# Circuitscape/Circuitscape.jl

Measured on NVIDIA H100. Metric: pair_solves_per_sec, higher is better.
Workload: dtype f64

## Files before the change

### circuitscape_b200/csrc/cs_b200.cu

```cuda
#include "../../include/cs_b200.h"

#include <cuda_runtime.h>
#include <cub/device/device_scan.cuh>

#include <algorithm>
#include <chrono>
#include <cmath>
#include <cstdarg>
#include <cstdio>
#include <cstdlib>
#include <cstring>
#include <limits>
#include <string>
#include <type_traits>
#include <vector>

#include "amg_host.hpp"
#include "win_host.hpp"
#include "kernels.cuh"
#include "raster_assembly.cuh"
#include "setup_device.hpp"

using namespace csb;

// ... 73 lines not shown
  bool mixed = false;
  std::vector<DevLevel> lv32;
  void *R32 = nullptr, *X32 = nullptr, *T32 = nullptr, *Z32 = nullptr;
  void *d_cum = nullptr, *d_max = nullptr;
  int* d_bptr = nullptr;
  int64_t nb = 0;
  void* d_cum_branch = nullptr;
  void* d_branch_stage = nullptr;
  PanelCtl* d_ctl = nullptr;
  PanelCtl* h_ctl = nullptr;
  double* d_partials = nullptr;
  float* d_flush = nullptr;
  size_t flush_elems = 0;
  cudaStream_t stream = nullptr;
  cudaEvent_t ev0 = nullptr, ev1 = nullptr, ev2 = nullptr, ev3 = nullptr;
  long long* d_sp_rows = nullptr;
  double* d_sp_vals = nullptr;
  int* d_sp_ptr = nullptr;
  size_t sp_cap = 0;
  long long* d_probe = nullptr;
  void* d_probe_out = nullptr;
  size_t probe_cap = 0;
  cudaStream_t s_in = nullptr, s_out = nullptr;
  void* io_in[2] = {nullptr, nullptr};
  void* io_out[2] = {nullptr, nullptr};
  cudaEvent_t ev_in[2] = {nullptr, nullptr}, ev_used[2] = {nullptr, nullptr};
  cudaEvent_t ev_ready[2] = {nullptr, nullptr}, ev_out[2] = {nullptr, nullptr};
  int num_sms = 132;
  int grid_spmm = 132, grid_ew = 132;
  cs_b200_opts opts{};
  cs_b200_stats stats{};
  GraphSlot graphs[4];
  bool rg_on = false;
  int* d_rg_seg = nullptr;
  int* d_rg_rows = nullptr;
  size_t rg_cap = 0;
  GraphSlot rgraphs[4];
  int profile = 0;
  std::vector<cudaEvent_t> prof_ev;
  size_t prof_used = 0;
  double prof_ms = 0.0;
  double prof_bytes = 0.0;
  int64_t prof_launches = 0;
  std::vector<int> prof_slot;
  std::vector<double> prof_pair_bytes;
  double prof_slot_ms[PROF_CLASSES] = {}, prof_slot_bytes[PROF_CLASSES] = {};
  int64_t prof_slot_launches[PROF_CLASSES] = {};
  std::string err;
  size_t esize() const { return dtype == CS_B200_F64 ? 8 : 4; }
};

namespace {

struct Tick {
  bool on = std::getenv("CS_B200_VERBOSE") != nullptr;
  std::chrono::steady_clock::time_point t0 = std::chrono::steady_clock::now();
  void operator()(const char* what) {
    if (!on) return;
    const auto t1 = std::chrono::steady_clock::now();
    std::fprintf(stderr, "[cs_b200 setup] %-28s %8.1f ms\n", what,
                 std::chrono::duration<double, std::milli>(t1 - t0).count());
    t0 = t1;
  }
};

int set_err(cs_b200_handle* h, int code, const char* fmt, ...) {
// ... 676 lines not shown

inline int copy_grid(size_t nelem) { return (int)std::min<size_t>(4096, (nelem + 255) / 256); }

template <typename T, int KT, int MODE, bool HALF>
void launch_stencil_pipe(cs_b200_handle* h, const DiaDev<T>& a, const T* X, T* Y, const SpmmEpi<T>& ep, int sg) {
  constexpr int SMEM = StPipe<T, KT, MODE, HALF>::D::BYTES;
  set_max_smem_once<k_stencil_pipe<T, KT, MODE, HALF>>(h, SMEM);
  k_stencil_pipe<T, KT, MODE, HALF><<<sg, NT, SMEM, h->stream>>>(a, X, Y, ep);
}

template <typename T, int KT, int MODE>
void launch_stencil(cs_b200_handle* h, const DiaDev<T>& a, const T* X, T* Y, const SpmmEpi<T>& ep, int sg) {
  if (!stencil_pipe()) {
    if (a.half) refuse_half("k_stencil");
    k_stencil<T, KT, MODE><<<sg, NT, 0, h->stream>>>(a, X, Y, ep);
    return;
  }
  if (a.half) launch_stencil_pipe<T, KT, MODE, true>(h, a, X, Y, ep, sg);
  else launch_stencil_pipe<T, KT, MODE, false>(h, a, X, Y, ep, sg);
}

template <typename T, int KT, int MODE, bool WIDE>
void launch_spmm_win(cs_b200_handle* h, const DevCsr& m, const T* X, T* Y, const SpmmEpi<T>& ep) {
  constexpr int SMEM = WinSmem2<T, KT, MODE, WIDE>::TOTAL;
  constexpr int SB = WinMap<T, KT, WIDE>::SB;
  const WinCsr<T> w{m.win_meta, m.blob, m.has_dinv, m.rowptr, m.colidx, (const T*)m.vals, m.win_nblocks};
  const int wg = std::max(1, std::min(h->num_sms, (m.win_nblocks + SB - 1) / SB));
  set_max_smem_once<k_spmm_win<T, KT, MODE, WIDE>>(h, SMEM);
  k_spmm_win<T, KT, MODE, WIDE><<<wg, WTT, SMEM, h->stream>>>(w, X, Y, ep);
}

template <typename T, int KT, int MODE>
void launch_spmm_on(cs_b200_handle* h, const DevCsr& m, const T* X, T* Y, const T* B, const T* dinv,
                    double omega, bool timed) {
  const int grid = std::max(1, std::min(h->grid_spmm, m.nblocks));
  double bytes = (double)m.nnz * (sizeof(T) + 4) + (double)(m.nrows + 1) * 4 +
                 2.0 * (double)m.nrows * KT * sizeof(T);
  if (MODE == SP_RESNORM || MODE == SP_RES || MODE == SP_JACOBI || MODE == SP_JACOBI_DOT)
    bytes += (double)m.nrows * KT * sizeof(T);
  if (MODE == SP_JACOBI || MODE == SP_JACOBI_DOT) bytes += (double)m.nrows * sizeof(T);
  const ProfScope prof(h, timed, MODE, sizeof(T) == 4, bytes);
  const SpmmEpi<T> ep{B, dinv, (T)omega, h->d_ctl, h->d_partials};
  if (m.dia && MODE != SP_ADD) {
    if constexpr (MODE != SP_ADD) launch_stencil<T, KT, MODE>(h, dia_view<T>(m), X, Y, ep, stencil_grid<T, KT>(h, m));
  } else if (m.win_meta) {
    if (m.lpr == 4) launch_spmm_win<T, KT, MODE, true>(h, m, X, Y, ep);
    else launch_spmm_win<T, KT, MODE, false>(h, m, X, Y, ep);
  } else if (m.lpr == 4 && KT * 4 <= 32) {
    k_spmm<T, KT, MODE, (KT * 4 <= 32 ? 4 : 1)><<<grid, NT, 0, h->stream>>>(view<T>(m), X, Y, ep);
  } else {
    k_spmm<T, KT, MODE, 1><<<grid, NT, 0, h->stream>>>(view<T>(m), X, Y, ep);
  }
}

template <typename T, int KT, int MODE>
void launch_spmm(cs_b200_handle* h, const T* X, T* Y, const T* B) {
  launch_spmm_on<T, KT, MODE>(h, h->A0, X, Y, B, (const T*)h->d_dinv, 0.0, true);
}

void harvest_profile(cs_b200_handle* h) {
  for (size_t i = 0; i + 1 < h->prof_used; i += 2) {
    float ms = 0;
    if (cudaEventElapsedTime(&ms, h->prof_ev[i], h->prof_ev[i + 1]) == cudaSuccess) {
      h->prof_ms += ms;
      h->prof_launches++;
      if (i / 2 < h->prof_slot.size()) {
        const int sl = h->prof_slot[i / 2];
        h->prof_slot_ms[sl] += ms;
        h->prof_slot_bytes[sl] += h->prof_pair_bytes[i / 2];
        h->prof_slot_launches[sl]++;
      }
    }
  }
  h->prof_used = 0;
  h->prof_slot.clear();
// ... 108 lines not shown

template <typename T, int KT>
void launch_seg_set(cs_b200_handle* h, void* panel, int set_b_only, T v) {
  k_seg_set<T, KT><<<2 * KT, NT, 0, h->stream>>>((T*)panel, h->d_rg_seg, h->d_rg_rows, set_b_only, v);
  h->stats.kernel_launches++;
}

template <typename T, int KT>
void mask_z(cs_b200_handle* h) {
  if (!h->rg_on) return;
  if (h->mixed) launch_seg_set<float, KT>(h, h->Z32, 0, 0.0f);
  else launch_seg_set<T, KT>(h, h->Z, 0, T(0));
}

inline GraphSlot& graph_slot(cs_b200_handle* h, int kt) {
  return (h->rg_on ? h->rgraphs : h->graphs)[kt_index(kt)];
}

void drop_graphs(GraphSlot* slots) {
  for (int i = 0; i < 4; ++i) {
    if (slots[i].exec) cudaGraphExecDestroy(slots[i].exec);
    if (slots[i].loop_exec) cudaGraphExecDestroy(slots[i].loop_exec);
    slots[i] = GraphSlot{};
  }
}

inline bool fused_cg(const cs_b200_handle* h) {
  static const bool off = std::getenv("CS_B200_NO_FUSED_CG") != nullptr;
  return h->amg && h->A0.dia && h->P2 && !off;
}

inline bool fused_res(const cs_b200_handle* h) {
  return fused_cg(h) && h->R2 && !h->rg_on && fused_res_form(h);
}

template <typename T, int KT, typename TV, bool HALF, bool STORE_AP>
void launch_stencil_cg_pipe(cs_b200_handle* h, const DiaDev<T>& a, const TV* Z, int sg) {
  constexpr int SMEM = StPipeCg<T, KT, TV, HALF>::D::BYTES;
  set_max_smem_once<k_stencil_cg_pipe<T, KT, TV, HALF, STORE_AP>>(h, SMEM);
  k_stencil_cg_pipe<T, KT, TV, HALF, STORE_AP><<<sg, NT, SMEM, h->stream>>>(a, Z, (T*)h->P2, (T*)h->P, (T*)h->X,
                                                                            (T*)h->AP, h->d_ctl, h->d_partials);
}

template <typename T, int KT, typename TV>
void launch_stencil_cg(cs_b200_handle* h, const TV* Z, bool store_ap) {
  const DevCsr& m = h->A0;
  const DiaDev<T> a = dia_view<T>(m);
  const int sg = stencil_grid<T, KT>(h, m);
  const double pe = (double)m.nrows * KT * sizeof(T);
  const double fb = (double)m.nrows * 9 * sizeof(T) + (double)m.nrows * KT * sizeof(TV) + (store_ap ? 3.0 : 2.0) * pe +
                    1.5 * pe;
  const ProfScope prof(h, true, PROF_CGF, sizeof(T) == 4, fb);
  if (stencil_pipe()) {
    if (!store_ap) {
      if constexpr (sizeof(T) == 8 && sizeof(TV) == 4) launch_stencil_cg_pipe<T, KT, TV, true, false>(h, a, Z, sg);
    } else if (a.half) launch_stencil_cg_pipe<T, KT, TV, true, true>(h, a, Z, sg);
    else launch_stencil_cg_pipe<T, KT, TV, false, true>(h, a, Z, sg);
  } else {
    if (a.half) refuse_half("k_stencil_cg");
    k_stencil_cg<T, KT, TV><<<sg, NT, 0, h->stream>>>(a, Z, (T*)h->P2, (T*)h->P, (T*)h->X, (T*)h->AP, h->d_ctl,
                                                       h->d_partials);
  }
}

template <typename T, int KT>
void launch_res_update(cs_b200_handle* h) {
// ... 133 lines not shown
    const int64_t kl = h->stats.kernel_launches, sl = h->stats.spmm_launches;
    CK(h, cudaStreamBeginCaptureToGraph(h->stream, body, nullptr, nullptr, 0, cudaStreamCaptureModeThreadLocal));
    launch_iteration<T, KT>(h);
    k_loop_cond<<<1, 1, 0, h->stream>>>(cond, h->d_ctl);
    CK(h, cudaStreamEndCapture(h->stream, nullptr));
    gs.loop_kernels = h->stats.kernel_launches - kl + 1;
    gs.loop_spmms = h->stats.spmm_launches - sl;
    h->stats.kernel_launches = kl;
    h->stats.spmm_launches = sl;
    CK(h, cudaGraphInstantiate(&gs.loop_exec, graph, 0));
    cudaGraphDestroy(graph);
  }
  CK(h, cudaGraphLaunch(gs.loop_exec, h->stream));
  return CS_B200_OK;
}

template <typename T, int KT>
int solve_panel(cs_b200_handle* h, double rtol, int64_t itmax) {
  const size_t nelem = (size_t)h->n_pad * KT;
  const double atol = h->opts.atol > 0 ? h->opts.atol
                      : h->opts.atol < 0 ? 0.0
                      : std::sqrt(std::numeric_limits<double>::epsilon());
  const int g = ew_grid<T, KT>(h);
  const int imax = (int)std::min<int64_t>(itmax, std::numeric_limits<int>::max() - 1);
  CK(h, cudaEventRecord(h->ev2, h->stream));
  if (!h->amg) {
    k_set_stall<<<1, 1, 0, h->stream>>>(h->d_ctl, 2000);
    k_cg_init<T, KT><<<g, NT, 0, h->stream>>>(nelem, (const T*)h->B, (const T*)h->d_dinv, (T*)h->X,
                                              (T*)h->R, (T*)h->P, h->d_ctl, h->d_partials, rtol, atol,
                                              imax);
    h->stats.kernel_launches++;
  } else {
    const bool fused = fused_cg(h);
    CK(h, cudaMemsetAsync(h->X, 0, nelem * sizeof(T), h->stream));
    CK(h, cudaMemsetAsync(h->P, 0, nelem * sizeof(T), h->stream));
    CK(h, cudaMemcpyAsync(h->R, h->B, nelem * sizeof(T), cudaMemcpyDeviceToDevice, h->stream));
    k_set_ctl<<<1, 1, 0, h->stream>>>(h->d_ctl, rtol, atol, imax, 40);
    h->stats.kernel_launches++;
    if (h->mixed) {
      k_convert<T, float><<<g, NT, 0, h->stream>>>(nelem, (const T*)h->R, (float*)h->R32);
      h->stats.kernel_launches++;
    }
    launch_vcycle<T, KT>(h, false);
    mask_z<T, KT>(h);
    if (!fused) launch_update_xp2<T, KT>(h);
  }
  CK(h, cudaGetLastError());
  const int chunk = h->amg ? std::min(h->opts.check_every, 4) : h->opts.check_every;
  const bool device_loop = h->opts.use_graph == 1 && !h->profile;
  if (device_loop) {
    int rc = run_loop<T, KT>(h);
    if (rc) return rc;
  }
  for (;;) {
    CK(h, cudaMemcpyAsync(h->h_ctl, h->d_ctl, sizeof(PanelCtl), cudaMemcpyDeviceToHost, h->stream));
    CK(h, cudaStreamSynchronize(h->stream));
    if (h->profile) harvest_profile(h);
    if (device_loop) {
      GraphSlot& gs = graph_slot(h, KT);
      h->stats.kernel_launches += 1 + gs.loop_kernels * h->h_ctl->iter;
      h->stats.spmm_launches += gs.loop_spmms * h->h_ctl->iter;
      break;
    }
    if (h->h_ctl->nactive == 0) break;
    int rc = run_chunk<T, KT>(h, chunk);
    if (rc) return rc;
  }
  if (h->amg) finish_x<T, KT>(h);
  if (h->rg_on) {
    launch_spmm<T, KT, SP_RES>(h, (const T*)h->X, (T*)h->AP, (const T*)h->B);
    launch_seg_set<T, KT>(h, h->AP, 0, T(0));
    k_resnorm<T, KT><<<g, NT, 0, h->stream>>>(nelem, (size_t)h->n * KT, (const T*)h->AP, (const T*)h->B, h->d_ctl, h->d_partials);
    h->stats.kernel_launches++;
  } else {
    launch_spmm<T, KT, 2>(h, (const T*)h->X, (T*)h->AP, (const T*)h->B);
  }
  CK(h, cudaGetLastError());
  CK(h, cudaEventRecord(h->ev3, h->stream));
  CK(h, cudaMemcpyAsync(h->h_ctl, h->d_ctl, sizeof(PanelCtl), cudaMemcpyDeviceToHost, h->stream));
  CK(h, cudaStreamSynchronize(h->stream));
  if (h->profile) harvest_profile(h);
  float ms = 0;
  CK(h, cudaEventElapsedTime(&ms, h->ev2, h->ev3));
  h->stats.kernel_ms += ms;
  return CS_B200_OK;
}

int next_kt(int64_t remaining, int ktmax) {
  int kt = ktmax;
  while (kt > remaining) kt >>= 1;
  return kt < 1 ? 1 : kt;
}

#define DISPATCH_KT(kt, CALL)                    \
  switch (kt) {                                  \
    case 1: { constexpr int KT = 1; CALL; } break; \
    case 2: { constexpr int KT = 2; CALL; } break; \
    case 4: { constexpr int KT = 4; CALL; } break; \
    default: { constexpr int KT = 8; CALL; } break; \
  }

template <typename F>
decltype(auto) with_type(const cs_b200_handle* h, F&& f) {
  return h->dtype == CS_B200_F64 ? f(double{}) : f(float{});
}

template <typename F>
decltype(auto) with_width(int kt, F&& f) {
  DISPATCH_KT(kt, return f(std::integral_constant<int, KT>{}));
}

template <typename F>
decltype(auto) with_type_width(const cs_b200_handle* h, int kt, F&& f) {
  return with_type(h, [&](auto t) -> decltype(auto) {
    return with_width(kt, [&](auto KT) -> decltype(auto) { return f(t, KT); });
  });
}

struct ColumnDriver {
  cs_b200_handle* h;
  bool any_fail = false, any_maxit = false;
  std::string msg;

  template <typename Panel>
  int run(int64_t c_begin, int64_t c_end, Panel&& panel) {
    for (int64_t c0 = c_begin; c0 < c_end;) {
      const int kt = next_kt(c_end - c0, h->ktmax);
      if (int rc = with_width(kt, [&](auto KT) { return panel(KT, c0); })) return rc;
      c0 += kt;
    }
    return CS_B200_OK;
  }

  template <typename T, int KT>
  int solve(int64_t c0, double rtol, int64_t itmax, int64_t* iters, double* relres, bool masked = false) {
    h->rg_on = masked;
    const int rc = solve_panel<T, KT>(h, rtol, itmax);
    h->rg_on = false;
    if (!rc) gather(KT, c0, iters, relres, itmax);
    return rc;
  }

  void gather(int kt, int64_t c0, int64_t* iters, double* relres, int64_t itmax) {
    for (int c = 0; c < kt; ++c) {
      const PanelCtl& ct = *h->h_ctl;
      const double bn = ct.bnorm[c];
      const double rr = bn > 0 ? std::sqrt(ct.resid[c] / bn) : 0.0;
      if (iters) iters[c0 + c] = ct.iters[c];
      if (relres) relres[c0 + c] = rr;
      h->stats.iterations += ct.iters[c];
      if (!(rr < h->opts.resid_gate)) {
        if (!any_fail) {
          char buf[256];
          snprintf(buf, sizeof buf,
                   "CUDA PCG solver residual %g exceeds tolerance %g for column %lld (%d iterations)",
                   rr, h->opts.resid_gate, (long long)(c0 + c + 1), ct.iters[c]);
          msg = buf;
        }
        any_fail = true;
      }
      if ((ct.iters[c] >= itmax || ct.stalled[c]) && std::sqrt(ct.rho[c]) > ct.tol[c]) any_maxit = true;
    }
  }

  int verdict(int rc) const {
    if (rc) return rc;
    if (any_fail) return set_err(h, CS_B200_ERR_RESIDUAL, "%s", msg.c_str());
    if (any_maxit) return set_err(h, CS_B200_ERR_MAXITER, "itmax reached (or the recurrence stagnated) before rtol");
    return CS_B200_OK;
  }
};
// ... 122 lines not shown
  }
  CK(h, h2d(h, h->d_probe, probe, need * sizeof(long long)));
  return CS_B200_OK;
}

template <typename T, int KT>
int download_outputs(cs_b200_handle* h, int64_t c0, T* curr, T* volt, int volt_shift) {
  CK(h, cudaGetLastError());
  const int tg = copy_grid((size_t)h->n_pad * KT);
  auto download = [&](const void* panel, int shift, T* out) -> int {
    k_panel_to_cm<T, KT><<<tg, 256, 0, h->stream>>>((int)h->n, (size_t)h->n, (const T*)panel, (T*)h->stage,
                                                    h->d_ctl, shift);
    h->stats.kernel_launches++;
    CK(h, cudaMemcpyAsync(out + (size_t)c0 * h->n, h->stage, (size_t)h->n * KT * sizeof(T),
                          cudaMemcpyDeviceToHost, h->stream));
    h->stats.d2h_bytes += (double)h->n * KT * sizeof(T);
    return CS_B200_OK;
  };
  if (curr)
    if (int rc = download(h->AP, 0, curr)) return rc;
  if (volt)
    if (int rc = download(h->X, volt_shift, volt)) return rc;
  return CS_B200_OK;
}

template <typename T, int KT>
int currents_and_outputs(cs_b200_handle* h, int64_t c0, T* curr, T* volt, int accumulate, int volt_shift,
                         const void* fg = nullptr) {
  if (accumulate || curr) launch_currents<T, KT>(h, curr != nullptr, accumulate, fg);
  return download_outputs<T, KT>(h, c0, curr, volt, volt_shift);
}

template <typename T, int KT>
int pairs_panel(cs_b200_handle* h, int64_t c0, const int64_t* src, const int64_t* dst,
                const double* weight, double rtol, int64_t itmax, T* R, T* volt, T* curr,
                int accumulate, int64_t* iters, double* relres, ColumnDriver& cols) {
  if (int rc = upload_ctl(h, KT, [&](int c) {
        return ColCtl{src[c0 + c], dst[c0 + c], col_weight(weight, c0 + c)};
      }))
    return rc;
  CK(h, cudaMemsetAsync(h->B, 0, (size_t)h->n_pad * KT * sizeof(T), h->stream));
  k_pair_rhs<T, KT><<<1, 32, 0, h->stream>>>((T*)h->B, h->d_ctl);
  h->stats.kernel_launches++;
  if (int rc = cols.solve<T, KT>(c0, rtol, itmax, iters, relres)) return rc;
  k_pair_extract<T, KT><<<1, 32, 0, h->stream>>>((const T*)h->X, h->d_ctl);
  h->stats.kernel_launches++;
  if (int rc = currents_and_outputs<T, KT>(h, c0, curr, volt, accumulate, 1)) return rc;
  if (int rc = read_ctl(h)) return rc;
  for (int c = 0; c < KT; ++c) R[c0 + c] = (T)(h->h_ctl->xdst[c] - h->h_ctl->xsrc[c]);
  return CS_B200_OK;
}

template <typename T, int KT>
int sources_panel(cs_b200_handle* h, int64_t c0, const int64_t* colptr, const int64_t* rows,
                  const double* vals, const int64_t* ref, const double* weight, double rtol,
                  int64_t itmax, int64_t nprobe, T* probe_volt, T* volt, T* curr, int accumulate,
                  int64_t* iters, double* relres, ColumnDriver& cols) {
  if (int rc = upload_ctl(h, KT, [&](int c) { return ColCtl{ref[c0 + c], -1, col_weight(weight, c0 + c)}; }))
    return rc;
  if (int rc = upload_sparse_rhs(h, KT, colptr + c0, rows, vals)) return rc;
  CK(h, cudaMemsetAsync(h->B, 0, (size_t)h->n_pad * KT * sizeof(T), h->stream));
  k_sparse_rhs<T, KT><<<1, 32, 0, h->stream>>>((T*)h->B, h->d_sp_ptr, h->d_sp_rows, h->d_sp_vals);
  h->stats.kernel_launches++;
  if (int rc = cols.solve<T, KT>(c0, rtol, itmax, iters, relres)) return rc;
  k_pair_extract<T, KT><<<1, 32, 0, h->stream>>>((const T*)h->X, h->d_ctl);
  h->stats.kernel_launches++;
  if (nprobe > 0 && probe_volt) {
    k_probe<T, KT><<<(int)std::min<int64_t>(64, (nprobe * KT + 255) / 256), 256, 0, h->stream>>>(
        (const T*)h->X, h->d_ctl, h->d_probe, (int)nprobe, (T*)h->d_probe_out);
    h->stats.kernel_launches++;
    CK(h, cudaMemcpyAsync(probe_volt + (size_t)c0 * nprobe, h->d_probe_out, (size_t)nprobe * KT * sizeof(T),
                          cudaMemcpyDeviceToHost, h->stream));
    h->stats.d2h_bytes += (double)nprobe * KT * sizeof(T);
  }
  if (int rc = currents_and_outputs<T, KT>(h, c0, curr, volt, accumulate, 1)) return rc;
  CK(h, cudaStreamSynchronize(h->stream));
  return CS_B200_OK;
}

template <typename T, int KT>
int point_panel(cs_b200_handle* h, int64_t x0, const int64_t* nodes, double rtol, int64_t itmax, T* U,
                int64_t* point_iters, ColumnDriver& cols) {
  const size_t nelem = (size_t)h->n_pad * KT;
  if (int rc = upload_ctl(h, KT, [&](int c) { return ColCtl{nodes[0], nodes[x0 + c], 1.0}; })) return rc;
  CK(h, cudaMemsetAsync(h->B, 0, nelem * sizeof(T), h->stream));
  k_pair_rhs<T, KT><<<1, 32, 0, h->stream>>>((T*)h->B, h->d_ctl);
  h->stats.kernel_launches++;
  if (int rc = cols.solve<T, KT>(0, rtol, itmax, nullptr, nullptr)) return rc;
  if (point_iters)
    for (int c = 0; c < KT; ++c) point_iters[x0 - 1 + c] = h->h_ctl->iters[c];
  k_pair_extract<T, KT><<<1, 32, 0, h->stream>>>((const T*)h->X, h->d_ctl);
  const int tg = copy_grid(nelem);
  k_panel_to_cm<T, KT><<<tg, 256, 0, h->stream>>>((int)h->n, (size_t)h->n_pad, (const T*)h->X,
                                                  U + (size_t)(x0 - 1) * h->n_pad, h->d_ctl, 1);
  h->stats.kernel_launches += 2;
  CK(h, cudaGetLastError());
  CK(h, cudaStreamSynchronize(h->stream));
  return CS_B200_OK;
}

template <typename T, int KT>
int combine_panel(cs_b200_handle* h, int64_t c0, const int64_t* nodes, const int64_t* pi, const int64_t* pj,
                  const double* weight, const T* U, int* d_ci, int* d_cj, T* R, T* volt, T* curr,
                  int accumulate, double* relres, int64_t itmax, ColumnDriver& cols) {
  const size_t nelem = (size_t)h->n_pad * KT;
  if (int rc = upload_ctl(h, KT, [&](int c) {
        return ColCtl{nodes[pi[c0 + c]], nodes[pj[c0 + c]], col_weight(weight, c0 + c)};
      }))
    return rc;
  int ci[MAXKT], cj[MAXKT];
  for (int c = 0; c < KT; ++c) {
    ci[c] = (int)pi[c0 + c] - 1;
    cj[c] = (int)pj[c0 + c] - 1;
  }
  CK(h, h2d(h, d_ci, ci, KT * sizeof(int)));
  CK(h, h2d(h, d_cj, cj, KT * sizeof(int)));
  h->stats.h2d_bytes += 2.0 * KT * sizeof(int);
  const int tg = copy_grid(nelem);
  k_combine<T, KT><<<tg, 256, 0, h->stream>>>((int)h->n, (size_t)h->n_pad, U, d_ci, d_cj, (T*)h->X);
  CK(h, cudaMemsetAsync(h->B, 0, nelem * sizeof(T), h->stream));
// ... 1643 lines not shown
```

### circuitscape_b200/csrc/kernels.cuh

```cuda
#pragma once
#include <cuda_runtime.h>
#include <stdint.h>

namespace csb {

constexpr int NT = 256;
constexpr int NWARP = NT / 32;
constexpr int NNZ_CAP = 2304;
constexpr int MAXKT = 8;

struct PanelCtl {
  double rho[MAXKT];
  double pap[MAXKT];
  double alpha[MAXKT];
  double beta[MAXKT];
  double tol[MAXKT];
  double rho0[MAXKT];
  double resid[MAXKT];
  double bnorm[MAXKT];
  double xsrc[MAXKT];
  double xdst[MAXKT];
  double maxpos[MAXKT];
  double maxneg[MAXKT];
  double weight[MAXKT];
// ... 168 lines not shown
    ctl->nactive = na;
    ctl->iter = init ? 0 : it;
    ctl->init = 0;
  }
}

#define CSB_REDUCE_SMEM(NV, KT)                         \
  __shared__ double s_warp[NWARP * (NV) * (KT)];        \
  __shared__ double s_tree[NT];                         \
  __shared__ double s_out[(NV) * (KT)];
#define CSB_REDUCE_SMEM_W(NV, KT)                       \
  __shared__ double s_warp[(WTT / 32) * (NV) * (KT)];   \
  __shared__ double s_tree[WTT];                        \
  __shared__ double s_out[(NV) * (KT)];

enum { SP_PLAIN = 0, SP_CG = 1, SP_RESNORM = 2, SP_RES = 3, SP_JACOBI = 4, SP_JACOBI_DOT = 5, SP_ADD = 6,
       SP_RES0 = 7  };

template <typename T> struct CsrDev {
  const int* rowptr;
  const int* colidx;
  const T* vals;
  const int* bstart;
  int nblocks;
  int nrows;
};

template <typename T> struct SpmmEpi {
  const T* B;
  const T* dinv;
  T omega;
  PanelCtl* ctl;
  double* partials;
};

template <typename T, int MODE>
__device__ __forceinline__ void spmm_epilogue(int row, size_t o, T acc, const T* __restrict__ X,
                                              T* __restrict__ Y, const SpmmEpi<T>& ep, double& dot0,
                                              double& dot1) {
  if (MODE == SP_PLAIN) {
    Y[o] = acc;
  } else if (MODE == SP_CG) {
    Y[o] = acc;
    dot0 += (double)acc * (double)X[o];
  } else if (MODE == SP_RESNORM) {
    const T bb = ep.B[o];
    const T rr = bb - acc;
    Y[o] = rr;
    dot0 += (double)rr * (double)rr;
    dot1 += (double)bb * (double)bb;
  } else if (MODE == SP_RES) {
    Y[o] = ep.B[o] - acc;
  } else if (MODE == SP_JACOBI || MODE == SP_JACOBI_DOT) {
    const T bb = ep.B[o];
    const T yn = X[o] + ep.omega * ep.dinv[row] * (bb - acc);
    Y[o] = yn;
    if (MODE == SP_JACOBI_DOT) dot0 += (double)bb * (double)yn;
  } else {
    Y[o] += acc;
  }
}

template <typename T, int KT, int MODE, int LPR>
__global__ void __launch_bounds__(NT)
k_spmm(const CsrDev<T> A, const T* __restrict__ X, T* __restrict__ Y, const SpmmEpi<T> ep) {
  __shared__ T s_val[NNZ_CAP];
  __shared__ int s_col[NNZ_CAP];
// ... 794 lines not shown
template <typename T, int KT, typename TV>
__global__ void __launch_bounds__(NT, CGF_MINB)
k_stencil_cg(const DiaDev<T> A, const TV* __restrict__ Z, T* Pb0, T* Pb1, T* __restrict__ X, T* __restrict__ Y,
             PanelCtl* ctl, double* partials) {
  const int it = ctl->iter;
  stencil_cg_body<T, KT, TV>(A, Z, (it & 1) ? Pb0 : Pb1, (it & 1) ? Pb1 : Pb0, X, Y, ctl, partials, it);
}

constexpr int ST_SMAX = 4;
constexpr int st_a16(int b) { return (b + 15) & ~15; }

template <int PANEL, int OWN, int MINB, int EXTRA = 0> struct StDepth {
  static constexpr int BUDGET = 228 * 1024 / MINB - 1024 - 3 * 1024 - EXTRA;
  static constexpr int FIT = (BUDGET - 3 * PANEL - OWN) / (PANEL + OWN);
  static constexpr int S = FIT < 1 ? 1 : (FIT > ST_SMAX ? ST_SMAX : FIT);
  static constexpr int BYTES = (S + 3) * PANEL + (S + 1) * OWN + EXTRA;
};

template <int B>
__device__ __forceinline__ void cp_async_zfill(void* dst, const void* src, bool ok) {
  const int sz = ok ? B : 0;
  if constexpr (B == 16)
    asm volatile("cp.async.cg.shared.global [%0], [%1], 16, %2;" ::"r"(smem_u32(dst)), "l"(src), "r"(sz) : "memory");
  else
    asm volatile("cp.async.ca.shared.global [%0], [%1], %2, %3;" ::"r"(smem_u32(dst)), "l"(src), "n"(B), "r"(sz)
                 : "memory");
}
__device__ __forceinline__ void cp_async_commit() { asm volatile("cp.async.commit_group;" ::: "memory"); }
template <int N> __device__ __forceinline__ void cp_async_wait() {
  asm volatile("cp.async.wait_group %0;" ::"n"(N) : "memory");
}

template <typename U, int W, int NROWS>
__device__ __forceinline__ void cp_rows(U* dst, const U* src, long long g0, int n) {
  constexpr int RB = W * (int)sizeof(U);
  constexpr int CH = RB < 16 ? RB : 16;
  constexpr int CPR = RB / CH;
  constexpr int NCH = NROWS * CPR;
#pragma unroll 1
  for (int q0 = 0; q0 < NCH; q0 += NT) {
    const int q = q0 + (int)threadIdx.x;
    if (NCH % NT == 0 || q < NCH) {
      const long long g = g0 + q / CPR;
      const bool ok = g >= 0 && g < n;
      cp_async_zfill<CH>(reinterpret_cast<char*>(dst) + q * CH,
                         reinterpret_cast<const char*>(src + (ok ? g : 0) * W) + (q % CPR) * CH, ok);
    }
  }
}

template <typename T, int RPP>
__device__ __forceinline__ void cp_diag(T* dst, const DiaDev<T>& A, long long row0) {
  constexpr int NCH = 9 * RPP;
#pragma unroll 1
  for (int q0 = 0; q0 < NCH; q0 += NT) {
    const int q = q0 + (int)threadIdx.x;
    if (NCH % NT == 0 || q < NCH) {
      const long long g = row0 + q % RPP;
      const bool ok = g < A.n;
      cp_async_zfill<(int)sizeof(T)>(dst + q, A.run(q / RPP) + (ok ? g : 0), ok);
    }
  }
}

template <typename T, int RPP>
__device__ __forceinline__ void cp_diag_half(T* dst, const DiaDev<T>& A, long long g0, int u0, int u1) {
  constexpr int RW = RPP + 2;
  const int nch = (u1 - u0) * RW;
#pragma unroll 1
  for (int q = (int)threadIdx.x; q < nch; q += NT) {
    const int u = u0 + q / RW, rr = q % RW;
    const long long g = g0 + rr;
    const bool ok = g >= 0 && g < A.n;
    cp_async_zfill<(int)sizeof(T)>(dst + u * RW + rr, A.run(4 + u) + (ok ? g : 0), ok);
  }
}

// ... 86 lines not shown
};

template <typename T, int KT, int MODE, bool HALF>
__global__ void __launch_bounds__(NT, 3)
k_stencil_pipe(const DiaDev<T> A, const T* __restrict__ X, T* __restrict__ Y, const SpmmEpi<T> ep) {
  using SP = StPipe<T, KT, MODE, HALF>;
  constexpr int CPT = SP::CPT, RPP = SP::RPP, S = SP::D::S;
  constexpr int RP = S + 3;
  extern __shared__ __align__(128) unsigned char st_sm[];
  unsigned char* const pring = st_sm;
  unsigned char* const oring = st_sm + RP * SP::PANEL;
  const int tid = threadIdx.x;
  const int cg = tid % (KT / CPT), rl = tid / (KT / CPT), c0 = cg * CPT;
  const int n = A.n, nr = A.nr;
  double dot0[CPT], dot1[CPT];
#pragma unroll
  for (int i = 0; i < CPT; ++i) dot0[i] = dot1[i] = 0.0;

  const T* const G = MODE == SP_RES0 ? ep.B : X;
  auto issue = [&](const StStep& s, int lp, int lo) {
    unsigned char* ps = pring + lp * SP::PANEL;
    const long long g0 = (long long)s.c * nr + s.r0 - 1;
    cp_rows<T, KT, RPP + 2>(reinterpret_cast<T*>(ps), G, g0, n);
    if (MODE == SP_RES0) cp_rows<T, 1, RPP + 2>(reinterpret_cast<T*>(ps + SP::PX), ep.dinv, g0, n);
    if (HALF) {
      int u0, u1;
      s.half_runs(u0, u1);
      cp_diag_half<T, RPP>(reinterpret_cast<T*>(ps + SP::PDG), A, g0, u0, u1);
    }
    if (s.c > s.cs) {
      unsigned char* os = oring + lo * SP::OWN;
      const long long row0 = (long long)(s.c - 1) * nr + s.r0;
      if (!HALF) cp_diag<T, RPP>(reinterpret_cast<T*>(os), A, row0);
      if (SP::NEEDB) cp_rows<T, KT, RPP>(reinterpret_cast<T*>(os + SP::OD), ep.B, row0, n);
      if (SP::NEEDD) cp_rows<T, 1, RPP>(reinterpret_cast<T*>(os + SP::OD + SP::OB), ep.dinv, row0, n);
    }
  };
  auto compute = [&](const StStep& s, int sp, int so) {
    const int c = s.c - 1, r = s.r0 + rl;
    const long long row_l = (long long)c * nr + r;
    if (r >= nr || row_l >= n) return;
    const int row = (int)row_l;
    const T* xs[3];
    const T* ws[3];
    const T* ds[3];
#pragma unroll
    for (int d = 0; d < 3; ++d) {
      const int k = sp + d + RP - 2;
      const unsigned char* p = pring + (k >= RP ? k - RP : k) * SP::PANEL;
      xs[d] = reinterpret_cast<const T*>(p);
      ws[d] = reinterpret_cast<const T*>(p + SP::PX);
      ds[d] = reinterpret_cast<const T*>(p + SP::PDG);
    }
    const unsigned char* os = oring + so * SP::OWN;
    const T* dg = reinterpret_cast<const T*>(os);
    T acc[CPT], xo[CPT];
#pragma unroll
    for (int i = 0; i < CPT; ++i) acc[i] = T(0);
#pragma unroll
    for (int s9 = 0; s9 < 9; ++s9) {
      T xv[CPT];
      ldvec<T, CPT>(xs[s9 / 3] + (rl + s9 % 3) * KT + c0, xv);
      if (s9 == 4) {
#pragma unroll
        for (int i = 0; i < CPT; ++i) xo[i] = xv[i];
      }
      const T a9 = HALF ? st_half_val<T, RPP>(ds, s9, rl) : dg[s9 * RPP + rl];
      const T vs = MODE == SP_RES0 ? a9 * (ep.omega * ws[s9 / 3][rl + s9 % 3]) : a9;
#pragma unroll
      for (int i = 0; i < CPT; ++i) acc[i] += vs * xv[i];
    }
    const size_t o = (size_t)row * KT + c0;
    T out[CPT], bb[CPT];
    if (SP::NEEDB) ldvec<T, CPT>(reinterpret_cast<const T*>(os + SP::OD) + rl * KT + c0, bb);
    T dv = T(0);
    if (SP::NEEDD) dv = ep.omega * reinterpret_cast<const T*>(os + SP::OD + SP::OB)[rl];
#pragma unroll
    for (int i = 0; i < CPT; ++i) {
      if (MODE == SP_PLAIN) {
        out[i] = acc[i];
      } else if (MODE == SP_CG) {
        out[i] = acc[i];
        dot0[i] += (double)acc[i] * (double)xo[i];
      } else if (MODE == SP_RESNORM) {
        const T rr = bb[i] - acc[i];
        out[i] = rr;
        dot0[i] += (double)rr * (double)rr;
        dot1[i] += (double)bb[i] * (double)bb[i];
      } else if (MODE == SP_RES) {
        out[i] = bb[i] - acc[i];
      } else if (MODE == SP_RES0) {
        out[i] = xo[i] - acc[i];
      } else {
        const T yn = xo[i] + dv * (bb[i] - acc[i]);
        out[i] = yn;
        if (MODE == SP_JACOBI_DOT) dot0[i] += (double)bb[i] * (double)yn;
      }
    }
    stvec<T, CPT>(Y + o, out);
  };
  stencil_pipe<S, RPP>(n, nr, issue, compute);

  if (MODE == SP_CG) {
    CSB_REDUCE_SMEM(1, KT)
    double v[1][CPT];
#pragma unroll
    for (int i = 0; i < CPT; ++i) v[0][i] = dot0[i];
    if (grid_reduce<KT, CPT, 1, false>(v, ep.partials, &ep.ctl->ticket, s_warp, s_tree, s_out)) {
      if (tid < KT) {
        const double pap = s_out[tid];
        ep.ctl->pap[tid] = pap;
        ep.ctl->alpha[tid] = (ep.ctl->active[tid] && pap > 0.0) ? ep.ctl->rho[tid] / pap : 0.0;
      }
    }
  } else if (MODE == SP_RESNORM) {
    CSB_REDUCE_SMEM(2, KT)
    double v[2][CPT];
#pragma unroll
    for (int i = 0; i < CPT; ++i) { v[0][i] = dot0[i]; v[1][i] = dot1[i]; }
    if (grid_reduce<KT, CPT, 2, false>(v, ep.partials, &ep.ctl->ticket, s_warp, s_tree, s_out)) {
      if (tid < KT) {
        ep.ctl->resid[tid] = s_out[tid];
        ep.ctl->bnorm[tid] = s_out[KT + tid];
      }
    }
  } else if (MODE == SP_JACOBI_DOT) {
    CSB_REDUCE_SMEM(1, KT)
    double v[1][CPT];
#pragma unroll
    for (int i = 0; i < CPT; ++i) v[0][i] = dot0[i];
    if (grid_reduce<KT, CPT, 1, false>(v, ep.partials, &ep.ctl->ticket, s_warp, s_tree, s_out))
      cg_after_precond<KT>(ep.ctl, s_out);
// ... 2 lines not shown

constexpr int CGP_MINB = 3;

template <typename T, int KT, typename TV, bool HALF> struct StPipeCg {
  static constexpr int V16 = 16 / (int)sizeof(T);
  static constexpr int CPT = KT < V16 ? KT : V16;
  static constexpr int RPP = NT / (KT / CPT);
  static constexpr int PP = st_a16((RPP + 2) * KT * (int)sizeof(T));
  static constexpr int PDG = PP + st_a16((RPP + 2) * KT * (int)sizeof(TV));
  static constexpr int PANEL = PDG + (HALF ? st_a16(5 * (RPP + 2) * (int)sizeof(T)) : 0);
  static constexpr int OD = HALF ? 0 : st_a16(9 * RPP * (int)sizeof(T));
  static constexpr int OX = st_a16(RPP * KT * (int)sizeof(T));
  static constexpr int OWN = OD + 2 * OX;
  using D = StDepth<PANEL, OWN, CGP_MINB>;
};

template <typename T, int KT, typename TV, bool HALF, bool STORE_AP>
__global__ void __launch_bounds__(NT, CGP_MINB)
k_stencil_cg_pipe(const DiaDev<T> A, const TV* __restrict__ Z, T* Pb0, T* Pb1, T* __restrict__ X, T* __restrict__ Y,
                  PanelCtl* ctl, double* partials) {
  using SP = StPipeCg<T, KT, TV, HALF>;
  constexpr int CPT = SP::CPT, RPP = SP::RPP, S = SP::D::S;
  constexpr int RP = S + 3;
  extern __shared__ __align__(128) unsigned char st_sm[];
  unsigned char* const pring = st_sm;
  unsigned char* const oring = st_sm + RP * SP::PANEL;
  const int it = ctl->iter;
  const T* const Pold = (it & 1) ? Pb0 : Pb1;
  T* const Pd = (it & 1) ? Pb1 : Pb0;
  const int tid = threadIdx.x;
  const int cg = tid % (KT / CPT), rl = tid / (KT / CPT), c0 = cg * CPT;
  const int n = A.n, nr = A.nr;
  const bool pair = it & 1;
  T be[CPT], a1[CPT], a2[CPT];
#pragma unroll
  for (int i = 0; i < CPT; ++i) {
    be[i] = (T)ctl->beta[c0 + i];
    a1[i] = (T)ctl->alpha_ring[(it + 2) % 3][c0 + i];
    a2[i] = (T)ctl->alpha_ring[(it + 1) % 3][c0 + i];
  }
  double dot0[CPT];
#pragma unroll
  for (int i = 0; i < CPT; ++i) dot0[i] = 0.0;

  auto issue = [&](const StStep& s, int lp, int lo) {
    unsigned char* ps = pring + lp * SP::PANEL;
    const long long g0 = (long long)s.c * nr + s.r0 - 1;
    cp_rows<T, KT, RPP + 2>(reinterpret_cast<T*>(ps), Pold, g0, n);
    cp_rows<TV, KT, RPP + 2>(reinterpret_cast<TV*>(ps + SP::PP), Z, g0, n);
    if (HALF) {
      int u0, u1;
      s.half_runs(u0, u1);
      cp_diag_half<T, RPP>(reinterpret_cast<T*>(ps + SP::PDG), A, g0, u0, u1);
    }
    if (s.c > s.cs) {
      unsigned char* os = oring + lo * SP::OWN;
      const long long row0 = (long long)(s.c - 1) * nr + s.r0;
      if (!HALF) cp_diag<T, RPP>(reinterpret_cast<T*>(os), A, row0);
      if (pair) {
        cp_rows<T, KT, RPP>(reinterpret_cast<T*>(os + SP::OD), X, row0, n);
        cp_rows<T, KT, RPP>(reinterpret_cast<T*>(os + SP::OD + SP::OX), Pd, row0, n);
      }
    }
  };
  auto compute = [&](const StStep& s, int sp, int so) {
    const int c = s.c - 1, r = s.r0 + rl;
    const long long row_l = (long long)c * nr + r;
    if (r >= nr || row_l >= n) return;
    const int row = (int)row_l;
    const T* ps[3];
    const TV* zs[3];
    const T* ds[3];
#pragma unroll
    for (int d = 0; d < 3; ++d) {
      const int k = sp + d + RP - 2;
      const unsigned char* p = pring + (k >= RP ? k - RP : k) * SP::PANEL;
      ps[d] = reinterpret_cast<const T*>(p);
      zs[d] = reinterpret_cast<const TV*>(p + SP::PP);
      ds[d] = reinterpret_cast<const T*>(p + SP::PDG);
    }
    const unsigned char* os = oring + so * SP::OWN;
    const T* dg = reinterpret_cast<const T*>(os);
    T acc[CPT], po[CPT], pc[CPT];
    stencil_row<T, CPT>(
        acc,
        [&](int s9, T (&pv)[CPT]) {
          TV zv[CPT];
          ldvec<T, CPT>(ps[s9 / 3] + (rl + s9 % 3) * KT + c0, pv);
          ldvec<TV, CPT>(zs[s9 / 3] + (rl + s9 % 3) * KT + c0, zv);
          if (s9 == 4) {
#pragma unroll
            for (int i = 0; i < CPT; ++i) po[i] = pv[i];
          }
#pragma unroll
// ... 631 lines not shown
                const PanelCtl* ctl) {
  constexpr int VEC = Vec<T>::N;
  const size_t e0 = ((size_t)blockIdx.x * NT + threadIdx.x) * VEC;
  const size_t stride = (size_t)gridDim.x * NT * VEC;
  T al[VEC], be[VEC];
#pragma unroll
  for (int i = 0; i < VEC; ++i) {
    al[i] = (T)ctl->alpha[(e0 + i) % KT];
    be[i] = (T)ctl->beta[(e0 + i) % KT];
  }
  for (size_t e = e0; e < nelem; e += stride) {
    TV z[VEC];
    T p[VEC], x[VEC];
    ldvec<TV, VEC>(Z + e, z);
    vload(P + e, p);
    vload(X + e, x);
#pragma unroll
    for (int i = 0; i < VEC; ++i) {
      x[i] += al[i] * p[i];
      p[i] = (T)z[i] + be[i] * p[i];
    }
    vstore(X + e, x);
    vstore(P + e, p);
  }
}

template <typename T, int KT>
__global__ void __launch_bounds__(NT)
k_cg_x_tail(size_t nelem, const T* __restrict__ Pb0, const T* __restrict__ Pb1, T* __restrict__ X,
            const PanelCtl* ctl) {
  constexpr int VEC = Vec<T>::N;
  const int K = ctl->iter;
  const bool two = K & 1;
  const T* p2 = (K & 1) ? Pb1 : Pb0;
  const T* p1 = (K & 1) ? Pb0 : Pb1;
  const size_t e0 = ((size_t)blockIdx.x * NT + threadIdx.x) * VEC;
  const size_t stride = (size_t)gridDim.x * NT * VEC;
  T a1[VEC], a2[VEC];
#pragma unroll
  for (int i = 0; i < VEC; ++i) {
    a1[i] = (T)ctl->alpha_ring[(K + 2) % 3][(e0 + i) % KT];
    a2[i] = (T)ctl->alpha_ring[(K + 1) % 3][(e0 + i) % KT];
  }
  for (size_t e = e0; e < nelem; e += stride) {
    T x[VEC], q1[VEC], q2[VEC];
    vload(X + e, x);
    vload(p1 + e, q1);
    if (two) {
      vload(p2 + e, q2);
#pragma unroll
      for (int i = 0; i < VEC; ++i) x[i] += a2[i] * q2[i];
    }
#pragma unroll
    for (int i = 0; i < VEC; ++i) x[i] += a1[i] * q1[i];
    vstore(X + e, x);
  }
}

template <typename TI, typename TO>
__global__ void __launch_bounds__(NT)
k_convert(size_t nelem, const TI* __restrict__ in, TO* __restrict__ out) {
  for (size_t e = (size_t)blockIdx.x * NT + threadIdx.x; e < nelem; e += (size_t)gridDim.x * NT)
    out[e] = (TO)in[e];
}

template <typename T, int KT>
__global__ void __launch_bounds__(NT)
k_jacobi0(size_t nelem, const T* __restrict__ B, const T* __restrict__ dinv, T omega,
          T* __restrict__ X) {
  constexpr int VEC = Vec<T>::N;
  constexpr int L = Log2<KT>::v;
  const size_t stride = (size_t)gridDim.x * NT * VEC;
  for (size_t e = ((size_t)blockIdx.x * NT + threadIdx.x) * VEC; e < nelem; e += stride) {
    T b[VEC], x[VEC];
    vload(B + e, b);
#pragma unroll
    for (int i = 0; i < VEC; ++i) x[i] = omega * dinv[(e + i) >> L] * b[i];
    vstore(X + e, x);
  }
}

template <typename T, int KT>
__global__ void __launch_bounds__(NT)
k_coarse_dense(int n, const double* __restrict__ pinv, const T* __restrict__ B, T* __restrict__ X) {
  const int e = blockIdx.x * NT + threadIdx.x;
  if (e >= n * KT) return;
  const int i = e / KT, c = e % KT;
  const double* row = pinv + (size_t)i * n;
  double a0 = 0.0, a1 = 0.0, a2 = 0.0, a3 = 0.0;
  int j = 0;
  for (; j + 3 < n; j += 4) {
    a0 += row[j] * (double)B[(size_t)j * KT + c];
    a1 += row[j + 1] * (double)B[(size_t)(j + 1) * KT + c];
    a2 += row[j + 2] * (double)B[(size_t)(j + 2) * KT + c];
    a3 += row[j + 3] * (double)B[(size_t)(j + 3) * KT + c];
  }
// ... 533 lines not shown
```

Baseline: 145.0.

## Fuse panel start and end passes, synthesizing pair RHS on the fly

For pair solves, the dense RHS buffer B is no longer materialized with a memset and a scatter kernel. Its entries are computed from the src/dst control data wherever they are needed: in a new fused start kernel that writes R and the float copy R32, and in the final residual-norm stencil, which also skips storing AP. The separate memsets of X and P, the R copy and the conversion kernel are replaced by that single start kernel. The first CG iterations skip loading X and P, which are known to be zero. This removes several full-vector passes and launches per panel, at the cost of extra branching and per-element src/dst comparisons.

```diff
diff --git a/circuitscape_b200/csrc/cs_b200.cu b/circuitscape_b200/csrc/cs_b200.cu
--- a/circuitscape_b200/csrc/cs_b200.cu
+++ b/circuitscape_b200/csrc/cs_b200.cu
@@ -129,6 +129,7 @@
   cs_b200_stats stats{};
   GraphSlot graphs[4];
   bool rg_on = false;
+  bool pair_b = false;
   int* d_rg_seg = nullptr;
   int* d_rg_rows = nullptr;
   size_t rg_cap = 0;
@@ -871,15 +872,16 @@
 
 template <typename T, int KT, int MODE>
 void launch_spmm_on(cs_b200_handle* h, const DevCsr& m, const T* X, T* Y, const T* B, const T* dinv,
-                    double omega, bool timed) {
+                    double omega, bool timed, bool pair_b = false) {
   const int grid = std::max(1, std::min(h->grid_spmm, m.nblocks));
   double bytes = (double)m.nnz * (sizeof(T) + 4) + (double)(m.nrows + 1) * 4 +
                  2.0 * (double)m.nrows * KT * sizeof(T);
   if (MODE == SP_RESNORM || MODE == SP_RES || MODE == SP_JACOBI || MODE == SP_JACOBI_DOT)
     bytes += (double)m.nrows * KT * sizeof(T);
   if (MODE == SP_JACOBI || MODE == SP_JACOBI_DOT) bytes += (double)m.nrows * sizeof(T);
+  if (pair_b) bytes -= 2.0 * (double)m.nrows * KT * sizeof(T);
   const ProfScope prof(h, timed, MODE, sizeof(T) == 4, bytes);
-  const SpmmEpi<T> ep{B, dinv, (T)omega, h->d_ctl, h->d_partials};
+  const SpmmEpi<T> ep{B, dinv, (T)omega, h->d_ctl, h->d_partials, pair_b ? 1 : 0};
   if (m.dia && MODE != SP_ADD) {
     if constexpr (MODE != SP_ADD) launch_stencil<T, KT, MODE>(h, dia_view<T>(m), X, Y, ep, stencil_grid<T, KT>(h, m));
   } else if (m.win_meta) {
@@ -1054,6 +1056,11 @@
 
 inline bool fused_res(const cs_b200_handle* h) {
   return fused_cg(h) && h->R2 && !h->rg_on && fused_res_form(h);
+}
+
+inline bool panel_ends(const cs_b200_handle* h) {
+  static const bool off = std::getenv("CS_B200_NO_FUSED_PANEL_ENDS") != nullptr;
+  return !off && fused_cg(h) && stencil_pipe();
 }
 
 template <typename T, int KT, typename TV, bool HALF, bool STORE_AP>
@@ -1253,14 +1260,21 @@
     h->stats.kernel_launches++;
   } else {
     const bool fused = fused_cg(h);
-    CK(h, cudaMemsetAsync(h->X, 0, nelem * sizeof(T), h->stream));
-    CK(h, cudaMemsetAsync(h->P, 0, nelem * sizeof(T), h->stream));
-    CK(h, cudaMemcpyAsync(h->R, h->B, nelem * sizeof(T), cudaMemcpyDeviceToDevice, h->stream));
-    k_set_ctl<<<1, 1, 0, h->stream>>>(h->d_ctl, rtol, atol, imax, 40);
-    h->stats.kernel_launches++;
-    if (h->mixed) {
-      k_convert<T, float><<<g, NT, 0, h->stream>>>(nelem, (const T*)h->R, (float*)h->R32);
+    if (panel_ends(h)) {
+      k_set_ctl<<<1, 1, 0, h->stream>>>(h->d_ctl, rtol, atol, imax, 40);
+      k_panel_start<T, KT><<<g, NT, 0, h->stream>>>(nelem, h->pair_b ? nullptr : (const T*)h->B, (T*)h->R,
+                                                    h->mixed ? (float*)h->R32 : nullptr, h->d_ctl);
+      h->stats.kernel_launches += 2;
+    } else {
+      CK(h, cudaMemsetAsync(h->X, 0, nelem * sizeof(T), h->stream));
+      CK(h, cudaMemsetAsync(h->P, 0, nelem * sizeof(T), h->stream));
+      CK(h, cudaMemcpyAsync(h->R, h->B, nelem * sizeof(T), cudaMemcpyDeviceToDevice, h->stream));
+      k_set_ctl<<<1, 1, 0, h->stream>>>(h->d_ctl, rtol, atol, imax, 40);
       h->stats.kernel_launches++;
+      if (h->mixed) {
+        k_convert<T, float><<<g, NT, 0, h->stream>>>(nelem, (const T*)h->R, (float*)h->R32);
+        h->stats.kernel_launches++;
+      }
     }
     launch_vcycle<T, KT>(h, false);
     mask_z<T, KT>(h);
@@ -1294,7 +1308,8 @@
     k_resnorm<T, KT><<<g, NT, 0, h->stream>>>(nelem, (size_t)h->n * KT, (const T*)h->AP, (const T*)h->B, h->d_ctl, h->d_partials);
     h->stats.kernel_launches++;
   } else {
-    launch_spmm<T, KT, 2>(h, (const T*)h->X, (T*)h->AP, (const T*)h->B);
+    launch_spmm_on<T, KT, SP_RESNORM>(h, h->A0, (const T*)h->X, (T*)h->AP, (const T*)h->B, (const T*)h->d_dinv, 0.0,
+                                      true, h->pair_b);
   }
   CK(h, cudaGetLastError());
   CK(h, cudaEventRecord(h->ev3, h->stream));
@@ -1358,6 +1373,7 @@
     h->rg_on = masked;
     const int rc = solve_panel<T, KT>(h, rtol, itmax);
     h->rg_on = false;
+    h->pair_b = false;
     if (!rc) gather(KT, c0, iters, relres, itmax);
     return rc;
   }
@@ -1546,6 +1562,16 @@
 }
 
 template <typename T, int KT>
+int stage_pair_rhs(cs_b200_handle* h) {
+  h->pair_b = panel_ends(h);
+  if (h->pair_b) return CS_B200_OK;
+  CK(h, cudaMemsetAsync(h->B, 0, (size_t)h->n_pad * KT * sizeof(T), h->stream));
+  k_pair_rhs<T, KT><<<1, 32, 0, h->stream>>>((T*)h->B, h->d_ctl);
+  h->stats.kernel_launches++;
+  return CS_B200_OK;
+}
+
+template <typename T, int KT>
 int pairs_panel(cs_b200_handle* h, int64_t c0, const int64_t* src, const int64_t* dst,
                 const double* weight, double rtol, int64_t itmax, T* R, T* volt, T* curr,
                 int accumulate, int64_t* iters, double* relres, ColumnDriver& cols) {
@@ -1553,9 +1579,7 @@
         return ColCtl{src[c0 + c], dst[c0 + c], col_weight(weight, c0 + c)};
       }))
     return rc;
-  CK(h, cudaMemsetAsync(h->B, 0, (size_t)h->n_pad * KT * sizeof(T), h->stream));
-  k_pair_rhs<T, KT><<<1, 32, 0, h->stream>>>((T*)h->B, h->d_ctl);
-  h->stats.kernel_launches++;
+  if (int rc = stage_pair_rhs<T, KT>(h)) return rc;
   if (int rc = cols.solve<T, KT>(c0, rtol, itmax, iters, relres)) return rc;
   k_pair_extract<T, KT><<<1, 32, 0, h->stream>>>((const T*)h->X, h->d_ctl);
   h->stats.kernel_launches++;
@@ -1597,9 +1621,7 @@
                 int64_t* point_iters, ColumnDriver& cols) {
   const size_t nelem = (size_t)h->n_pad * KT;
   if (int rc = upload_ctl(h, KT, [&](int c) { return ColCtl{nodes[0], nodes[x0 + c], 1.0}; })) return rc;
-  CK(h, cudaMemsetAsync(h->B, 0, nelem * sizeof(T), h->stream));
-  k_pair_rhs<T, KT><<<1, 32, 0, h->stream>>>((T*)h->B, h->d_ctl);
-  h->stats.kernel_launches++;
+  if (int rc = stage_pair_rhs<T, KT>(h)) return rc;
   if (int rc = cols.solve<T, KT>(0, rtol, itmax, nullptr, nullptr)) return rc;
   if (point_iters)
     for (int c = 0; c < KT; ++c) point_iters[x0 - 1 + c] = h->h_ctl->iters[c];
diff --git a/circuitscape_b200/csrc/kernels.cuh b/circuitscape_b200/csrc/kernels.cuh
--- a/circuitscape_b200/csrc/kernels.cuh
+++ b/circuitscape_b200/csrc/kernels.cuh
@@ -224,7 +224,20 @@
   T omega;
   PanelCtl* ctl;
   double* partials;
+  int pair_b;
 };
+
+template <typename T>
+__host__ __device__ __forceinline__ T pair_rhs_val(const PanelCtl* ctl, long long row, int c) {
+  const long long s = ctl->src[c], d = ctl->dst[c];
+  if (s < 0 || d < 0 || s == d) return T(0);
+  return row == d ? T(1) : row == s ? T(-1) : T(0);
+}
+
+template <typename T, int KT>
+__host__ __device__ __forceinline__ T pair_rhs_at(const PanelCtl* ctl, size_t e) {
+  return pair_rhs_val<T>(ctl, (long long)(e / KT), (int)(e % KT));
+}
 
 template <typename T, int MODE>
 __device__ __forceinline__ void spmm_epilogue(int row, size_t o, T acc, const T* __restrict__ X,
@@ -1085,7 +1098,7 @@
 }
 
 template <typename U, int W, int NROWS>
-__device__ __forceinline__ void cp_rows(U* dst, const U* src, long long g0, int n) {
+__device__ __forceinline__ void cp_rows(U* dst, const U* src, long long g0, int n, bool live = true) {
   constexpr int RB = W * (int)sizeof(U);
   constexpr int CH = RB < 16 ? RB : 16;
   constexpr int CPR = RB / CH;
@@ -1095,7 +1108,7 @@
     const int q = q0 + (int)threadIdx.x;
     if (NCH % NT == 0 || q < NCH) {
       const long long g = g0 + q / CPR;
-      const bool ok = g >= 0 && g < n;
+      const bool ok = live && g >= 0 && g < n;
       cp_async_zfill<CH>(reinterpret_cast<char*>(dst) + q * CH,
                          reinterpret_cast<const char*>(src + (ok ? g : 0) * W) + (q % CPR) * CH, ok);
     }
@@ -1248,7 +1261,8 @@
       unsigned char* os = oring + lo * SP::OWN;
       const long long row0 = (long long)(s.c - 1) * nr + s.r0;
       if (!HALF) cp_diag<T, RPP>(reinterpret_cast<T*>(os), A, row0);
-      if (SP::NEEDB) cp_rows<T, KT, RPP>(reinterpret_cast<T*>(os + SP::OD), ep.B, row0, n);
+      if (SP::NEEDB && !(MODE == SP_RESNORM && ep.pair_b))
+        cp_rows<T, KT, RPP>(reinterpret_cast<T*>(os + SP::OD), ep.B, row0, n);
       if (SP::NEEDD) cp_rows<T, 1, RPP>(reinterpret_cast<T*>(os + SP::OD + SP::OB), ep.dinv, row0, n);
     }
   };
@@ -1288,7 +1302,12 @@
     }
     const size_t o = (size_t)row * KT + c0;
     T out[CPT], bb[CPT];
-    if (SP::NEEDB) ldvec<T, CPT>(reinterpret_cast<const T*>(os + SP::OD) + rl * KT + c0, bb);
+    if (MODE == SP_RESNORM && ep.pair_b) {
+#pragma unroll
+      for (int i = 0; i < CPT; ++i) bb[i] = pair_rhs_val<T>(ep.ctl, row, c0 + i);
+    } else if (SP::NEEDB) {
+      ldvec<T, CPT>(reinterpret_cast<const T*>(os + SP::OD) + rl * KT + c0, bb);
+    }
     T dv = T(0);
     if (SP::NEEDD) dv = ep.omega * reinterpret_cast<const T*>(os + SP::OD + SP::OB)[rl];
 #pragma unroll
@@ -1313,7 +1332,7 @@
         if (MODE == SP_JACOBI_DOT) dot0[i] += (double)bb[i] * (double)yn;
       }
     }
-    stvec<T, CPT>(Y + o, out);
+    if (!(MODE == SP_RESNORM && ep.pair_b)) stvec<T, CPT>(Y + o, out);
   };
   stencil_pipe<S, RPP>(n, nr, issue, compute);
 
@@ -1382,6 +1401,7 @@
   const int cg = tid % (KT / CPT), rl = tid / (KT / CPT), c0 = cg * CPT;
   const int n = A.n, nr = A.nr;
   const bool pair = it & 1;
+  const bool p_live = it != 0, x_live = it != 1;
   T be[CPT], a1[CPT], a2[CPT];
 #pragma unroll
   for (int i = 0; i < CPT; ++i) {
@@ -1396,7 +1416,7 @@
   auto issue = [&](const StStep& s, int lp, int lo) {
     unsigned char* ps = pring + lp * SP::PANEL;
     const long long g0 = (long long)s.c * nr + s.r0 - 1;
-    cp_rows<T, KT, RPP + 2>(reinterpret_cast<T*>(ps), Pold, g0, n);
+    cp_rows<T, KT, RPP + 2>(reinterpret_cast<T*>(ps), Pold, g0, n, p_live);
     cp_rows<TV, KT, RPP + 2>(reinterpret_cast<TV*>(ps + SP::PP), Z, g0, n);
     if (HALF) {
       int u0, u1;
@@ -1408,8 +1428,8 @@
       const long long row0 = (long long)(s.c - 1) * nr + s.r0;
       if (!HALF) cp_diag<T, RPP>(reinterpret_cast<T*>(os), A, row0);
       if (pair) {
-        cp_rows<T, KT, RPP>(reinterpret_cast<T*>(os + SP::OD), X, row0, n);
-        cp_rows<T, KT, RPP>(reinterpret_cast<T*>(os + SP::OD + SP::OX), Pd, row0, n);
+        cp_rows<T, KT, RPP>(reinterpret_cast<T*>(os + SP::OD), X, row0, n, x_live);
+        cp_rows<T, KT, RPP>(reinterpret_cast<T*>(os + SP::OD + SP::OX), Pd, row0, n, x_live);
       }
     }
   };
@@ -2107,6 +2127,7 @@
   constexpr int VEC = Vec<T>::N;
   const int K = ctl->iter;
   const bool two = K & 1;
+  const bool x_live = K > 1, p_live = K > 0;
   const T* p2 = (K & 1) ? Pb1 : Pb0;
   const T* p1 = (K & 1) ? Pb0 : Pb1;
   const size_t e0 = ((size_t)blockIdx.x * NT + threadIdx.x) * VEC;
@@ -2119,10 +2140,12 @@
   }
   for (size_t e = e0; e < nelem; e += stride) {
     T x[VEC], q1[VEC], q2[VEC];
-    vload(X + e, x);
-    vload(p1 + e, q1);
+#pragma unroll
+    for (int i = 0; i < VEC; ++i) x[i] = q1[i] = q2[i] = T(0);
+    if (x_live) vload(X + e, x);
+    if (p_live) vload(p1 + e, q1);
     if (two) {
-      vload(p2 + e, q2);
+      if (x_live) vload(p2 + e, q2);
 #pragma unroll
       for (int i = 0; i < VEC; ++i) x[i] += a2[i] * q2[i];
     }
@@ -2137,6 +2160,30 @@
 k_convert(size_t nelem, const TI* __restrict__ in, TO* __restrict__ out) {
   for (size_t e = (size_t)blockIdx.x * NT + threadIdx.x; e < nelem; e += (size_t)gridDim.x * NT)
     out[e] = (TO)in[e];
+}
+
+template <typename T, int KT>
+__global__ void __launch_bounds__(NT)
+k_panel_start(size_t nelem, const T* __restrict__ B, T* __restrict__ R, float* __restrict__ R32,
+              const PanelCtl* __restrict__ ctl) {
+  constexpr int VEC = Vec<T>::N;
+  const size_t stride = (size_t)gridDim.x * NT * VEC;
+  for (size_t e = ((size_t)blockIdx.x * NT + threadIdx.x) * VEC; e < nelem; e += stride) {
+    T r[VEC];
+    if (B) {
+      vload(B + e, r);
+    } else {
+#pragma unroll
+      for (int i = 0; i < VEC; ++i) r[i] = pair_rhs_at<T, KT>(ctl, e + i);
+    }
+    vstore(R + e, r);
+    if (R32) {
+      if constexpr (VEC == 2)
+        *reinterpret_cast<float2*>(R32 + e) = make_float2((float)r[0], (float)r[1]);
+      else
+        *reinterpret_cast<float4*>(R32 + e) = make_float4((float)r[0], (float)r[1], (float)r[2], (float)r[3]);
+    }
+  }
 }
 
 template <typename T, int KT>
diff --git a/profiles/run_panel_ends.py b/profiles/run_panel_ends.py
--- /dev/null
+++ b/profiles/run_panel_ends.py
@@ -0,0 +1,136 @@
+#!/usr/bin/env python
+import argparse
+import json
+import os
+import re
+import subprocess
+import sys
+import tempfile
+from collections import defaultdict
+
+ROOT = os.path.dirname(os.path.dirname(os.path.abspath(__file__)))
+sys.path.insert(0, ROOT)
+SWITCH = "CS_B200_NO_FUSED_PANEL_ENDS"
+
+
+def card():
+    try:
+        out = subprocess.run(["nvidia-smi", "--query-gpu=name,power.limit", "--format=csv,noheader"],
+                             capture_output=True, text=True, timeout=30).stdout.strip().splitlines()
+        name, pl = [s.strip() for s in out[0].split(",")]
+        return {"name": name, "power_limit": pl}
+    except Exception as e:
+        return {"name": None, "power_limit": None, "error": str(e)}
+
+
+def short(name):
+    name = name.replace("(anonymous namespace)::", "").replace("csb::", "")
+    name = re.sub(r"^void ", "", name)
+    depth, cut = 0, len(name)
+    for i, ch in enumerate(name):
+        if ch == "<":
+            depth += 1
+        elif ch == ">":
+            depth -= 1
+        elif ch == "(" and depth == 0 and i > 0:
+            cut = i
+            break
+    return name[:cut].replace(" ", "")
+
+
+def child(rows, npairs, trace_path):
+    import numpy as np
+    import torch
+    from torch.profiler import ProfilerActivity, profile
+    import circuitscape_b200 as cb
+    from circuitscape_b200 import graph
+
+    L, _ = graph.synthetic_raster_laplacian(rows, rows, seed=42)
+    npts = 2
+    while npts * (npts - 1) // 2 < 128:
+        npts += 1
+    src, dst = graph.all_pairs(graph.focal_nodes(L.shape[0], npts, seed=7), limit=128)
+    src, dst = src[:npairs], dst[:npairs]
+    with cb.construct_cholesky_factor(L, cb.CUDASolver()) as f:
+        f.reset_currents()
+        f.solve_pairs(src, dst, accumulate=True)
+        torch.cuda.synchronize()
+        f.reset_currents()
+        with profile(activities=[ProfilerActivity.CUDA]) as prof:
+            out = f.solve_pairs(src, dst, accumulate=True)
+            torch.cuda.synchronize()
+        prof.export_chrome_trace(trace_path)
+        np.save(trace_path + ".R.npy", np.asarray(out["R"]))
+
+
+def panels(trace_path):
+    with open(trace_path) as fh:
+        ev = json.load(fh)["traceEvents"]
+    dev = sorted((e for e in ev if e.get("ph") == "X" and e.get("cat") in ("kernel", "gpu_memset", "gpu_memcpy")),
+                 key=lambda e: e["ts"])
+    out, cur = [], []
+    for e in dev:
+        cur.append(e)
+        if short(e["name"]).startswith("k_cur_acc_dia"):
+            out.append(cur)
+            cur = []
+    res = []
+    for p in out:
+        conds = [i for i, e in enumerate(p) if short(e["name"]).startswith("k_loop_cond")]
+        if not conds:
+            raise SystemExit("no k_loop_cond in a panel: the device WHILE loop did not run")
+        start, end = p[:conds[0]], p[conds[-1] + 1:]
+
+        def passes(seg):
+            agg = defaultdict(lambda: [0, 0.0])
+            for e in seg:
+                k = short(e["name"])
+                agg[k][0] += 1
+                agg[k][1] += e["dur"] / 1000.0
+            return [{"pass": k, "launches": n, "ms": round(ms, 4)} for k, (n, ms) in agg.items()]
+
+        res.append({"start_ms": round(sum(e["dur"] for e in start) / 1000.0, 4),
+                    "end_ms": round(sum(e["dur"] for e in end) / 1000.0, 4),
+                    "loop_cond_kernels": len(conds),
+                    "start": passes(start), "end": passes(end)})
+    return res
+
+
+def main():
+    ap = argparse.ArgumentParser()
+    ap.add_argument("--rows", type=int, default=3163)
+    ap.add_argument("--pairs", type=int, default=16)
+    ap.add_argument("--out", default=None)
+    ap.add_argument("--child", default=None, help=argparse.SUPPRESS)
+    a = ap.parse_args()
+    if a.child:
+        child(a.rows, a.pairs, a.child)
+        return
+    import numpy as np
+    result = {"card": card(), "rows": a.rows, "pairs": a.pairs, "settings": {}}
+    with tempfile.TemporaryDirectory() as tmp:
+        R = {}
+        for name, off in (("on", False), ("off", True)):
+            env = dict(os.environ)
+            env.pop(SWITCH, None)
+            if off:
+                env[SWITCH] = "1"
+            trace = os.path.join(tmp, f"{name}.json")
+            subprocess.run([sys.executable, os.path.abspath(__file__), "--rows", str(a.rows), "--pairs", str(a.pairs),
+                            "--child", trace], env=env, check=True, cwd=ROOT)
+            ps = panels(trace)
+            R[name] = np.load(trace + ".R.npy")
+            result["settings"][name] = {
+                "start_ms_per_panel": round(sum(p["start_ms"] for p in ps) / len(ps), 4),
+                "end_ms_per_panel": round(sum(p["end_ms"] for p in ps) / len(ps), 4),
+                "panels": ps}
+        result["R_identical"] = bool(np.array_equal(R["on"], R["off"]))
+    line = json.dumps(result)
+    print(line)
+    if a.out:
+        with open(a.out, "w") as fh:
+            fh.write(line + "\n")
+
+
+if __name__ == "__main__":
+    main()
```

Measured after the change: 150.8 (median of 6 runs). +4.0%, better.
